# zai-org/SCAIL

Hardware: NVIDIA H100
Metric: denoising steps/sec (SCAIL-14B, 512p/81f) (higher is better)
Workload: dtype bf16

## Files before the change

### scail_b200/csrc/attention.cuh

```cuda
#pragma once
#include "sm90.cuh"

namespace scail {

constexpr int ATT_D = 128;
constexpr int ATT_BQ = 128;
constexpr int ATT_BKV = 128;
constexpr int ATT_STAGES = 2;
constexpr int ATT_TILE_BYTES = 128 * 128 * 2;
constexpr int ATT_HALF_BYTES = ATT_TILE_BYTES / 2;
constexpr int ATT_THREADS = 384;
constexpr int ATT_SMEM_BYTES = (1 + 2 * ATT_STAGES) * ATT_TILE_BYTES + 1024 + 256;
static_assert(ATT_SMEM_BYTES <= 232448, "attention: shared memory budget");

struct AttnParams {
    __nv_bfloat16* out;
    int64_t ldo;
    int q_len;
    int kv_len;
    int kv_off;
    int kv_off1, kv_len1;
    float* o32;
    int64_t ldo32;
    float2* state;
    int heads;
    int q_batch_rows;
    int kv_batch_rows;
    float scale_log2;
    int accumulate;
};


__global__ void __launch_bounds__(ATT_THREADS, 1)
attention_fwd_kernel(const __grid_constant__ CUtensorMap tmap_q, const __grid_constant__ CUtensorMap tmap_k,
                     const __grid_constant__ CUtensorMap tmap_v, const AttnParams p) {
    extern __shared__ uint8_t smem_raw[];
    const uint32_t smem_base = (smem_u32(smem_raw) + 1023u) & ~1023u;
    const uint32_t q_smem = smem_base;
    const uint32_t k_smem = smem_base + ATT_TILE_BYTES;
    const uint32_t v_smem = k_smem + ATT_STAGES * ATT_TILE_BYTES;
    const uint32_t bar_base = v_smem + ATT_STAGES * ATT_TILE_BYTES;
    enum {
        B_QFULL = 0,
        B_KFULL = 1,
        B_KEMPTY = B_KFULL + ATT_STAGES,
        B_VFULL = B_KEMPTY + ATT_STAGES,
        B_VEMPTY = B_VFULL + ATT_STAGES,
        B_COUNT = B_VEMPTY + ATT_STAGES
    };
    static_assert(8 * B_COUNT <= 256, "attention: barrier area");
    auto bar = [&](int i) { return bar_base + 8u * i; };

    const int warp = threadIdx.x >> 5;
    const int lane = threadIdx.x & 31;
    const int head = blockIdx.y;
    const int batch = blockIdx.z;
    const int q0 = blockIdx.x * ATT_BQ;
    const int n_kv0 = (p.kv_len + ATT_BKV - 1) / ATT_BKV;
    const int n_kv = n_kv0 + (p.kv_len1 + ATT_BKV - 1) / ATT_BKV;

    if (warp == 0 && lane == 0) {
        tma_prefetch_desc(&tmap_q);
        tma_prefetch_desc(&tmap_k);
        tma_prefetch_desc(&tmap_v);
        mbar_init(bar(B_QFULL), 1);
        for (int s = 0; s < ATT_STAGES; ++s) {
            mbar_init(bar(B_KFULL + s), 1);
            mbar_init(bar(B_KEMPTY + s), 2);
            mbar_init(bar(B_VFULL + s), 1);
            mbar_init(bar(B_VEMPTY + s), 2);
        }
        fence_barrier_init();
    }
    __syncthreads();

    if (warp < 4) {
        setmaxnreg_dec<40>();
        if (warp == 0 && lane == 0) {
            const int col = head * ATT_D;
            mbar_expect_tx(bar(B_QFULL), ATT_TILE_BYTES);
            for (int h = 0; h < 2; ++h)
                tma_load_2d(q_smem + h * ATT_HALF_BYTES, &tmap_q, bar(B_QFULL), col + h * 64, batch * p.q_batch_rows + q0);
            const int kvbase = batch * p.kv_batch_rows;
            auto kv_row = [&](int j) { return kvbase + (j < n_kv0 ? p.kv_off + j * ATT_BKV : p.kv_off1 + (j - n_kv0) * ATT_BKV); };
            for (int j = 0; j < n_kv; ++j) {
                const int s = j % ATT_STAGES;
                const uint32_t par = ((j / ATT_STAGES) & 1) ^ 1;
                mbar_wait(bar(B_KEMPTY + s), par, 10);
                mbar_expect_tx(bar(B_KFULL + s), ATT_TILE_BYTES);
                for (int h = 0; h < 2; ++h)
                    tma_load_2d(k_smem + s * ATT_TILE_BYTES + h * ATT_HALF_BYTES, &tmap_k, bar(B_KFULL + s), col + h * 64, kv_row(j));
                mbar_wait(bar(B_VEMPTY + s), par, 11);
                mbar_expect_tx(bar(B_VFULL + s), ATT_TILE_BYTES);
                for (int h = 0; h < 2; ++h)
                    tma_load_2d(v_smem + s * ATT_TILE_BYTES + h * ATT_HALF_BYTES, &tmap_v, bar(B_VFULL + s), col + h * 64, kv_row(j));
            }
        }
    } else {
        setmaxnreg_inc<232>();
        const int wg = (warp >> 2) - 1;
        const int t = threadIdx.x & 127;
        const bool releaser = t == 0;
        const int quad = t & 3;
        float m_run[2] = {-INFINITY, -INFINITY};
        float l_run[2] = {0.f, 0.f};
        float o[ATT_D / 2];
#pragma unroll
        for (int i = 0; i < ATT_D / 2; ++i) o[i] = 0.f;
        const uint64_t q_desc = wgmma_desc_kmajor_sw128(q_smem + wg * (64 * 128));
        mbar_wait(bar(B_QFULL), 0, 20);
#pragma unroll 1
        for (int j = 0; j < n_kv; ++j) {
            const int s = j % ATT_STAGES;
            const uint32_t par = (j / ATT_STAGES) & 1;
            const int valid = j < n_kv0 ? min(ATT_BKV, p.kv_len - j * ATT_BKV) : min(ATT_BKV, p.kv_len1 - (j - n_kv0) * ATT_BKV);
            float sc[ATT_BKV / 2];
            mbar_wait(bar(B_KFULL + s), par, 21);
            const uint64_t k_desc = wgmma_desc_kmajor_sw128(k_smem + s * ATT_TILE_BYTES);
            wgmma_fence();
#pragma unroll
            for (int k = 0; k < 8; ++k) {
                const uint64_t off = ((k >> 2) * ATT_HALF_BYTES + (k & 3) * 32) >> 4;
                wgmma_ss<ATT_BKV>(sc, q_desc + off, k_desc + off, k != 0);
            }
            wgmma_commit();
            wgmma_wait<0>();
            fence_regs(sc);
            if (releaser) mbar_arrive(bar(B_KEMPTY + s));
            if (valid < ATT_BKV) {
#pragma unroll
                for (int c = 0; c < ATT_BKV / 8; ++c) {
                    const int col = 8 * c + 2 * quad;
                    if (col >= valid) { sc[4 * c] = -INFINITY; sc[4 * c + 2] = -INFINITY; }
                    if (col + 1 >= valid) { sc[4 * c + 1] = -INFINITY; sc[4 * c + 3] = -INFINITY; }
                }
            }
            float alpha[2], neg_m[2];
#pragma unroll
            for (int h = 0; h < 2; ++h) {
                float mx = -INFINITY;
#pragma unroll
                for (int c = 0; c < ATT_BKV / 8; ++c) mx = fmaxf(mx, fmaxf(sc[4 * c + 2 * h], sc[4 * c + 2 * h + 1]));
                mx = fmaxf(mx, __shfl_xor_sync(0xffffffffu, mx, 1));
                mx = fmaxf(mx, __shfl_xor_sync(0xffffffffu, mx, 2));
                const float m_new = fmaxf(m_run[h], mx * p.scale_log2);
                alpha[h] = fast_exp2(m_run[h] - m_new);
                m_run[h] = m_new;
                l_run[h] *= alpha[h];
                neg_m[h] = -m_new;
            }
#pragma unroll
            for (int c = 0; c < ATT_D / 8; ++c) {
                o[4 * c] *= alpha[0];
                o[4 * c + 1] *= alpha[0];
                o[4 * c + 2] *= alpha[1];
                o[4 * c + 3] *= alpha[1];
            }
            uint32_t pa[ATT_BKV / 16][4];
#pragma unroll
            for (int c = 0; c < ATT_BKV / 8; ++c) {
                float e[4];
#pragma unroll
                for (int i = 0; i < 4; ++i) {
                    e[i] = fast_exp2(fmaf(sc[4 * c + i], p.scale_log2, neg_m[i >> 1]));
                    l_run[i >> 1] += e[i];
                }
                pa[c >> 1][(c & 1) * 2] = pack_bf16(e[0], e[1]);
                pa[c >> 1][(c & 1) * 2 + 1] = pack_bf16(e[2], e[3]);
            }
            mbar_wait(bar(B_VFULL + s), par, 22);
            const uint64_t v_desc = wgmma_desc_mnmajor_sw128(v_smem + s * ATT_TILE_BYTES, ATT_HALF_BYTES);
            fence_regs(o);
            wgmma_fence();
#pragma unroll
            for (int k = 0; k < ATT_BKV / 16; ++k) wgmma_rs_tb<ATT_D>(o, pa[k], v_desc + k * (2048 >> 4));
            wgmma_commit();
            wgmma_wait<0>();
            fence_regs(o);
            if (releaser) mbar_arrive(bar(B_VEMPTY + s));
        }
#pragma unroll
        for (int h = 0; h < 2; ++h) {
            l_run[h] += __shfl_xor_sync(0xffffffffu, l_run[h], 1);
            l_run[h] += __shfl_xor_sync(0xffffffffu, l_run[h], 2);
        }
#pragma unroll
        for (int h = 0; h < 2; ++h) {
            const int qi = q0 + wg * 64 + (t >> 5) * 16 + ((t & 31) >> 2) + 8 * h;
            if (qi >= p.q_len) continue;
            const float inv_l = 1.0f / l_run[h];
            const int64_t grow = static_cast<int64_t>(batch) * p.q_batch_rows + qi;
            if (p.o32 != nullptr) {
                if (quad == 0) p.state[grow * p.heads + head] = make_float2(m_run[h], l_run[h]);
                float* dst = p.o32 + grow * p.ldo32 + head * ATT_D + 2 * quad;
#pragma unroll
                for (int c = 0; c < ATT_D / 8; ++c)
                    *reinterpret_cast<float2*>(dst + 8 * c) = make_float2(o[4 * c + 2 * h] * inv_l, o[4 * c + 2 * h + 1] * inv_l);
                continue;
            }
            __nv_bfloat16* dst = p.out + grow * p.ldo + head * ATT_D + 2 * quad;
#pragma unroll
            for (int c = 0; c < ATT_D / 8; ++c) {
                float f0 = o[4 * c + 2 * h] * inv_l, f1 = o[4 * c + 2 * h + 1] * inv_l;
                uint32_t* d32 = reinterpret_cast<uint32_t*>(dst + 8 * c);
                if (p.accumulate) {
                    const float2 prev = unpack_bf16(*d32);
                    f0 += prev.x;
                    f1 += prev.y;
                }
                *d32 = pack_bf16(f0, f1);
            }
        }
    }
}

__global__ void __launch_bounds__(256) attn_merge_kernel(const float* __restrict__ oa, const float2* __restrict__ sa,
                                                         const float* __restrict__ ob, const float2* __restrict__ sb,
                                                         __nv_bfloat16* __restrict__ out, int64_t ld32, int64_t ldo, int64_t rows,
                                                         int heads) {
    const int64_t item = (static_cast<int64_t>(blockIdx.x) * blockDim.x + threadIdx.x) >> 5;
    if (item >= rows * heads) return;
    const int lane = threadIdx.x & 31;
    const int64_t row = item / heads;
    const int head = static_cast<int>(item - row * heads);
    const float2 a = sa[item], b = sb[item];
    const float m = fmaxf(a.x, b.x);
    const float wa = a.y * fast_exp2(a.x - m), wb = b.y * fast_exp2(b.x - m);
    const float inv = 1.0f / (wa + wb);
    const float ca = wa * inv, cb = wb * inv;
    const float4 va = *reinterpret_cast<const float4*>(oa + row * ld32 + head * ATT_D + lane * 4);
    const float4 vb = *reinterpret_cast<const float4*>(ob + row * ld32 + head * ATT_D + lane * 4);
    uint2 o;
    o.x = pack_bf16(ca * va.x + cb * vb.x, ca * va.y + cb * vb.y);
    o.y = pack_bf16(ca * va.z + cb * vb.z, ca * va.w + cb * vb.w);
    *reinterpret_cast<uint2*>(out + row * ldo + head * ATT_D + lane * 4) = o;
}

}
```

### scail_b200/csrc/sm90.cuh

```cuda
#pragma once
#include <cuda.h>
#include <cuda_bf16.h>
#include <cuda_runtime.h>
#include <stdint.h>
#include <stdio.h>

namespace scail {

__device__ __forceinline__ uint32_t smem_u32(const void* p) {
    return static_cast<uint32_t>(__cvta_generic_to_shared(p));
}

__device__ __forceinline__ uint64_t global_timer_ns() {
    uint64_t t;
    asm volatile("mov.u64 %0, %%globaltimer;" : "=l"(t));
    return t;
}

__device__ __forceinline__ void mbar_init(uint32_t bar, uint32_t count) {
    asm volatile("mbarrier.init.shared::cta.b64 [%0], %1;" ::"r"(bar), "r"(count));
}
__device__ __forceinline__ void fence_barrier_init() {
    asm volatile("fence.mbarrier_init.release.cluster;" ::: "memory");
}
__device__ __forceinline__ void mbar_expect_tx(uint32_t bar, uint32_t bytes) {
    asm volatile("mbarrier.arrive.expect_tx.shared::cta.b64 _, [%0], %1;" ::"r"(bar), "r"(bytes) : "memory");
}
__device__ __forceinline__ void mbar_arrive(uint32_t bar) {
    asm volatile("mbarrier.arrive.shared::cta.b64 _, [%0];" ::"r"(bar) : "memory");
}
__device__ __forceinline__ bool mbar_try_wait(uint32_t bar, uint32_t parity) {
    uint32_t done;
    asm volatile(
        "{\n\t.reg .pred p;\n\t"
        "mbarrier.try_wait.parity.shared::cta.b64 p, [%1], %2;\n\t"
        "selp.b32 %0, 1, 0, p;\n\t}"
        : "=r"(done) : "r"(bar), "r"(parity) : "memory");
    return done != 0;
}
#ifndef SCAIL_MBAR_TIMEOUT_NS
#define SCAIL_MBAR_TIMEOUT_NS 4000000000ull
#endif
__device__ __forceinline__ void mbar_wait(uint32_t bar, uint32_t parity, int tag = 0) {
    if (mbar_try_wait(bar, parity)) return;
    uint64_t t0 = 0;
    uint32_t it = 0;
    while (!mbar_try_wait(bar, parity)) {
        if ((++it & 0x3ff) == 0) {
            uint64_t now = global_timer_ns();
            if (t0 == 0) t0 = now;
            else if (now - t0 > SCAIL_MBAR_TIMEOUT_NS) {
#ifdef SCAIL_MBAR_DEBUG
                printf("scail: mbarrier timeout tag=%d block=(%d,%d,%d) thread=%d parity=%u\n", tag, blockIdx.x,
                       blockIdx.y, blockIdx.z, threadIdx.x, parity);
#endif
                __trap();
            }
        }
    }
}

__device__ __forceinline__ void tma_prefetch_desc(const CUtensorMap* m) {
    asm volatile("prefetch.tensormap [%0];" ::"l"(reinterpret_cast<uint64_t>(m)) : "memory");
}
__device__ __forceinline__ void tma_load_2d(uint32_t dst, const CUtensorMap* m, uint32_t bar, int c0, int c1) {
    asm volatile(
        "cp.async.bulk.tensor.2d.shared::cluster.global.mbarrier::complete_tx::bytes [%0], [%1, {%3, %4}], [%2];"
        ::"r"(dst), "l"(reinterpret_cast<uint64_t>(m)), "r"(bar), "r"(c0), "r"(c1) : "memory");
}
__device__ __forceinline__ void tma_load_4d(uint32_t dst, const CUtensorMap* m, uint32_t bar, int c0, int c1, int c2,
                                            int c3) {
    asm volatile(
        "cp.async.bulk.tensor.4d.shared::cluster.global.mbarrier::complete_tx::bytes [%0], [%1, {%3, %4, %5, %6}], [%2];"
        ::"r"(dst), "l"(reinterpret_cast<uint64_t>(m)), "r"(bar), "r"(c0), "r"(c1), "r"(c2), "r"(c3) : "memory");
}
__device__ __forceinline__ void tma_store_2d(const CUtensorMap* m, uint32_t src, int c0, int c1) {
    asm volatile("cp.async.bulk.tensor.2d.global.shared::cta.bulk_group [%0, {%2, %3}], [%1];"
                 ::"l"(reinterpret_cast<uint64_t>(m)), "r"(src), "r"(c0), "r"(c1) : "memory");
}
__device__ __forceinline__ void bulk_commit() { asm volatile("cp.async.bulk.commit_group;" ::: "memory"); }
__device__ __forceinline__ void bulk_wait_read_all() { asm volatile("cp.async.bulk.wait_group.read 0;" ::: "memory"); }
__device__ __forceinline__ void bulk_wait_all() { asm volatile("cp.async.bulk.wait_group 0;" ::: "memory"); }
__device__ __forceinline__ void fence_proxy_async_smem() { asm volatile("fence.proxy.async.shared::cta;" ::: "memory"); }
__device__ __forceinline__ uint32_t lds_u32(uint32_t a) {
    uint32_t v;
    asm volatile("ld.shared.b32 %0, [%1];" : "=r"(v) : "r"(a) : "memory");
    return v;
}
__device__ __forceinline__ float2 lds_f2(uint32_t a) {
    float2 v;
    asm volatile("ld.shared.v2.f32 {%0, %1}, [%2];" : "=f"(v.x), "=f"(v.y) : "r"(a) : "memory");
    return v;
}
__device__ __forceinline__ void sts_u32(uint32_t a, uint32_t v) {
    asm volatile("st.shared.b32 [%0], %1;" ::"r"(a), "r"(v) : "memory");
}
__device__ __forceinline__ void sts_f2(uint32_t a, float x, float y) {
    asm volatile("st.shared.v2.f32 [%0], {%1, %2};" ::"r"(a), "f"(x), "f"(y) : "memory");
}

__device__ __forceinline__ uint64_t wgmma_desc_kmajor_sw128(uint32_t smem_addr) {
    uint64_t d = 0;
    d |= static_cast<uint64_t>((smem_addr & 0x3FFFFu) >> 4);
    d |= static_cast<uint64_t>(1) << 16;
    d |= static_cast<uint64_t>(1024 >> 4) << 32;
    d |= static_cast<uint64_t>(1) << 62;
    return d;
}
__device__ __forceinline__ uint64_t wgmma_desc_mnmajor_sw128(uint32_t smem_addr, uint32_t lbo_bytes) {
    uint64_t d = 0;
    d |= static_cast<uint64_t>((smem_addr & 0x3FFFFu) >> 4);
    d |= static_cast<uint64_t>((lbo_bytes >> 4) & 0x3FFFu) << 16;
    d |= static_cast<uint64_t>(1024 >> 4) << 32;
    d |= static_cast<uint64_t>(1) << 62;
    return d;
}
__device__ __forceinline__ void wgmma_fence() { asm volatile("wgmma.fence.sync.aligned;" ::: "memory"); }
__device__ __forceinline__ void wgmma_commit() { asm volatile("wgmma.commit_group.sync.aligned;" ::: "memory"); }
template <int N>
__device__ __forceinline__ void wgmma_wait() { asm volatile("wgmma.wait_group.sync.aligned %0;" ::"n"(N) : "memory"); }
template <int R>
__device__ __forceinline__ void fence_regs(float (&d)[R]) {
#pragma unroll
    for (int i = 0; i < R; ++i) asm volatile("" : "+f"(d[i])::"memory");
}

template <int N>
__device__ __forceinline__ void wgmma_ss(float (&d)[N / 2], uint64_t a, uint64_t b, int scale_d);
template <int N>
__device__ __forceinline__ void wgmma_rs_tb(float (&d)[N / 2], const uint32_t (&a)[4], uint64_t b);
template <>
__device__ __forceinline__ void wgmma_ss<16>(float (&d)[8], uint64_t a, uint64_t b, int scale_d) {
    asm volatile(
        "{\n\t.reg .pred p;\n\tsetp.ne.b32 p, %10, 0;\n\t"
        "wgmma.mma_async.sync.aligned.m64n16k16.f32.bf16.bf16 {%0, %1, %2, %3, %4, %5, %6, %7}, %8, %9, p, 1, 1, 0, 0;\n\t}"
        : "+f"(d[0]), "+f"(d[1]), "+f"(d[2]), "+f"(d[3]), "+f"(d[4]), "+f"(d[5]), "+f"(d[6]), "+f"(d[7])
        : "l"(a), "l"(b), "r"(scale_d));
}
template <>
__device__ __forceinline__ void wgmma_ss<96>(float (&d)[48], uint64_t a, uint64_t b, int scale_d) {
    asm volatile(
        "{\n\t.reg .pred p;\n\tsetp.ne.b32 p, %50, 0;\n\t"
        "wgmma.mma_async.sync.aligned.m64n96k16.f32.bf16.bf16 {%0, %1, %2, %3, %4, %5, %6, %7, %8, %9, %10, %11, %12, %13, %14, %15, %16, %17, %18, %19, %20, %21, %22, %23, %24, %25, %26, %27, %28, %29, %30, %31, %32, %33, %34, %35, %36, %37, %38, %39, %40, %41, %42, %43, %44, %45, %46, %47}, %48, %49, p, 1, 1, 0, 0;\n\t}"
        : "+f"(d[0]), "+f"(d[1]), "+f"(d[2]), "+f"(d[3]), "+f"(d[4]), "+f"(d[5]), "+f"(d[6]), "+f"(d[7]), "+f"(d[8]), "+f"(d[9]), "+f"(d[10]), "+f"(d[11]), "+f"(d[12]), "+f"(d[13]), "+f"(d[14]), "+f"(d[15]), "+f"(d[16]), "+f"(d[17]), "+f"(d[18]), "+f"(d[19]), "+f"(d[20]), "+f"(d[21]), "+f"(d[22]), "+f"(d[23]), "+f"(d[24]), "+f"(d[25]), "+f"(d[26]), "+f"(d[27]), "+f"(d[28]), "+f"(d[29]), "+f"(d[30]), "+f"(d[31]), "+f"(d[32]), "+f"(d[33]), "+f"(d[34]), "+f"(d[35]), "+f"(d[36]), "+f"(d[37]), "+f"(d[38]), "+f"(d[39]), "+f"(d[40]), "+f"(d[41]), "+f"(d[42]), "+f"(d[43]), "+f"(d[44]), "+f"(d[45]), "+f"(d[46]), "+f"(d[47])
        : "l"(a), "l"(b), "r"(scale_d));
}
template <>
__device__ __forceinline__ void wgmma_ss<128>(float (&d)[64], uint64_t a, uint64_t b, int scale_d) {
    asm volatile(
        "{\n\t.reg .pred p;\n\tsetp.ne.b32 p, %66, 0;\n\t"
        "wgmma.mma_async.sync.aligned.m64n128k16.f32.bf16.bf16 {%0, %1, %2, %3, %4, %5, %6, %7, %8, %9, %10, %11, %12, %13, %14, %15, %16, %17, %18, %19, %20, %21, %22, %23, %24, %25, %26, %27, %28, %29, %30, %31, %32, %33, %34, %35, %36, %37, %38, %39, %40, %41, %42, %43, %44, %45, %46, %47, %48, %49, %50, %51, %52, %53, %54, %55, %56, %57, %58, %59, %60, %61, %62, %63}, %64, %65, p, 1, 1, 0, 0;\n\t}"
        : "+f"(d[0]), "+f"(d[1]), "+f"(d[2]), "+f"(d[3]), "+f"(d[4]), "+f"(d[5]), "+f"(d[6]), "+f"(d[7]), "+f"(d[8]), "+f"(d[9]), "+f"(d[10]), "+f"(d[11]), "+f"(d[12]), "+f"(d[13]), "+f"(d[14]), "+f"(d[15]), "+f"(d[16]), "+f"(d[17]), "+f"(d[18]), "+f"(d[19]), "+f"(d[20]), "+f"(d[21]), "+f"(d[22]), "+f"(d[23]), "+f"(d[24]), "+f"(d[25]), "+f"(d[26]), "+f"(d[27]), "+f"(d[28]), "+f"(d[29]), "+f"(d[30]), "+f"(d[31]), "+f"(d[32]), "+f"(d[33]), "+f"(d[34]), "+f"(d[35]), "+f"(d[36]), "+f"(d[37]), "+f"(d[38]), "+f"(d[39]), "+f"(d[40]), "+f"(d[41]), "+f"(d[42]), "+f"(d[43]), "+f"(d[44]), "+f"(d[45]), "+f"(d[46]), "+f"(d[47]), "+f"(d[48]), "+f"(d[49]), "+f"(d[50]), "+f"(d[51]), "+f"(d[52]), "+f"(d[53]), "+f"(d[54]), "+f"(d[55]), "+f"(d[56]), "+f"(d[57]), "+f"(d[58]), "+f"(d[59]), "+f"(d[60]), "+f"(d[61]), "+f"(d[62]), "+f"(d[63])
        : "l"(a), "l"(b), "r"(scale_d));
}
template <>
__device__ __forceinline__ void wgmma_ss<192>(float (&d)[96], uint64_t a, uint64_t b, int scale_d) {
    asm volatile(
        "{\n\t.reg .pred p;\n\tsetp.ne.b32 p, %98, 0;\n\t"
        "wgmma.mma_async.sync.aligned.m64n192k16.f32.bf16.bf16 {%0, %1, %2, %3, %4, %5, %6, %7, %8, %9, %10, %11, %12, %13, %14, %15, %16, %17, %18, %19, %20, %21, %22, %23, %24, %25, %26, %27, %28, %29, %30, %31, %32, %33, %34, %35, %36, %37, %38, %39, %40, %41, %42, %43, %44, %45, %46, %47, %48, %49, %50, %51, %52, %53, %54, %55, %56, %57, %58, %59, %60, %61, %62, %63, %64, %65, %66, %67, %68, %69, %70, %71, %72, %73, %74, %75, %76, %77, %78, %79, %80, %81, %82, %83, %84, %85, %86, %87, %88, %89, %90, %91, %92, %93, %94, %95}, %96, %97, p, 1, 1, 0, 0;\n\t}"
        : "+f"(d[0]), "+f"(d[1]), "+f"(d[2]), "+f"(d[3]), "+f"(d[4]), "+f"(d[5]), "+f"(d[6]), "+f"(d[7]), "+f"(d[8]), "+f"(d[9]), "+f"(d[10]), "+f"(d[11]), "+f"(d[12]), "+f"(d[13]), "+f"(d[14]), "+f"(d[15]), "+f"(d[16]), "+f"(d[17]), "+f"(d[18]), "+f"(d[19]), "+f"(d[20]), "+f"(d[21]), "+f"(d[22]), "+f"(d[23]), "+f"(d[24]), "+f"(d[25]), "+f"(d[26]), "+f"(d[27]), "+f"(d[28]), "+f"(d[29]), "+f"(d[30]), "+f"(d[31]), "+f"(d[32]), "+f"(d[33]), "+f"(d[34]), "+f"(d[35]), "+f"(d[36]), "+f"(d[37]), "+f"(d[38]), "+f"(d[39]), "+f"(d[40]), "+f"(d[41]), "+f"(d[42]), "+f"(d[43]), "+f"(d[44]), "+f"(d[45]), "+f"(d[46]), "+f"(d[47]), "+f"(d[48]), "+f"(d[49]), "+f"(d[50]), "+f"(d[51]), "+f"(d[52]), "+f"(d[53]), "+f"(d[54]), "+f"(d[55]), "+f"(d[56]), "+f"(d[57]), "+f"(d[58]), "+f"(d[59]), "+f"(d[60]), "+f"(d[61]), "+f"(d[62]), "+f"(d[63]), "+f"(d[64]), "+f"(d[65]), "+f"(d[66]), "+f"(d[67]), "+f"(d[68]), "+f"(d[69]), "+f"(d[70]), "+f"(d[71]), "+f"(d[72]), "+f"(d[73]), "+f"(d[74]), "+f"(d[75]), "+f"(d[76]), "+f"(d[77]), "+f"(d[78]), "+f"(d[79]), "+f"(d[80]), "+f"(d[81]), "+f"(d[82]), "+f"(d[83]), "+f"(d[84]), "+f"(d[85]), "+f"(d[86]), "+f"(d[87]), "+f"(d[88]), "+f"(d[89]), "+f"(d[90]), "+f"(d[91]), "+f"(d[92]), "+f"(d[93]), "+f"(d[94]), "+f"(d[95])
        : "l"(a), "l"(b), "r"(scale_d));
}
template <>
__device__ __forceinline__ void wgmma_ss<256>(float (&d)[128], uint64_t a, uint64_t b, int scale_d) {
    asm volatile(
        "{\n\t.reg .pred p;\n\tsetp.ne.b32 p, %130, 0;\n\t"
        "wgmma.mma_async.sync.aligned.m64n256k16.f32.bf16.bf16 {%0, %1, %2, %3, %4, %5, %6, %7, %8, %9, %10, %11, %12, %13, %14, %15, %16, %17, %18, %19, %20, %21, %22, %23, %24, %25, %26, %27, %28, %29, %30, %31, %32, %33, %34, %35, %36, %37, %38, %39, %40, %41, %42, %43, %44, %45, %46, %47, %48, %49, %50, %51, %52, %53, %54, %55, %56, %57, %58, %59, %60, %61, %62, %63, %64, %65, %66, %67, %68, %69, %70, %71, %72, %73, %74, %75, %76, %77, %78, %79, %80, %81, %82, %83, %84, %85, %86, %87, %88, %89, %90, %91, %92, %93, %94, %95, %96, %97, %98, %99, %100, %101, %102, %103, %104, %105, %106, %107, %108, %109, %110, %111, %112, %113, %114, %115, %116, %117, %118, %119, %120, %121, %122, %123, %124, %125, %126, %127}, %128, %129, p, 1, 1, 0, 0;\n\t}"
        : "+f"(d[0]), "+f"(d[1]), "+f"(d[2]), "+f"(d[3]), "+f"(d[4]), "+f"(d[5]), "+f"(d[6]), "+f"(d[7]), "+f"(d[8]), "+f"(d[9]), "+f"(d[10]), "+f"(d[11]), "+f"(d[12]), "+f"(d[13]), "+f"(d[14]), "+f"(d[15]), "+f"(d[16]), "+f"(d[17]), "+f"(d[18]), "+f"(d[19]), "+f"(d[20]), "+f"(d[21]), "+f"(d[22]), "+f"(d[23]), "+f"(d[24]), "+f"(d[25]), "+f"(d[26]), "+f"(d[27]), "+f"(d[28]), "+f"(d[29]), "+f"(d[30]), "+f"(d[31]), "+f"(d[32]), "+f"(d[33]), "+f"(d[34]), "+f"(d[35]), "+f"(d[36]), "+f"(d[37]), "+f"(d[38]), "+f"(d[39]), "+f"(d[40]), "+f"(d[41]), "+f"(d[42]), "+f"(d[43]), "+f"(d[44]), "+f"(d[45]), "+f"(d[46]), "+f"(d[47]), "+f"(d[48]), "+f"(d[49]), "+f"(d[50]), "+f"(d[51]), "+f"(d[52]), "+f"(d[53]), "+f"(d[54]), "+f"(d[55]), "+f"(d[56]), "+f"(d[57]), "+f"(d[58]), "+f"(d[59]), "+f"(d[60]), "+f"(d[61]), "+f"(d[62]), "+f"(d[63]), "+f"(d[64]), "+f"(d[65]), "+f"(d[66]), "+f"(d[67]), "+f"(d[68]), "+f"(d[69]), "+f"(d[70]), "+f"(d[71]), "+f"(d[72]), "+f"(d[73]), "+f"(d[74]), "+f"(d[75]), "+f"(d[76]), "+f"(d[77]), "+f"(d[78]), "+f"(d[79]), "+f"(d[80]), "+f"(d[81]), "+f"(d[82]), "+f"(d[83]), "+f"(d[84]), "+f"(d[85]), "+f"(d[86]), "+f"(d[87]), "+f"(d[88]), "+f"(d[89]), "+f"(d[90]), "+f"(d[91]), "+f"(d[92]), "+f"(d[93]), "+f"(d[94]), "+f"(d[95]), "+f"(d[96]), "+f"(d[97]), "+f"(d[98]), "+f"(d[99]), "+f"(d[100]), "+f"(d[101]), "+f"(d[102]), "+f"(d[103]), "+f"(d[104]), "+f"(d[105]), "+f"(d[106]), "+f"(d[107]), "+f"(d[108]), "+f"(d[109]), "+f"(d[110]), "+f"(d[111]), "+f"(d[112]), "+f"(d[113]), "+f"(d[114]), "+f"(d[115]), "+f"(d[116]), "+f"(d[117]), "+f"(d[118]), "+f"(d[119]), "+f"(d[120]), "+f"(d[121]), "+f"(d[122]), "+f"(d[123]), "+f"(d[124]), "+f"(d[125]), "+f"(d[126]), "+f"(d[127])
        : "l"(a), "l"(b), "r"(scale_d));
}
template <>
__device__ __forceinline__ void wgmma_rs_tb<128>(float (&d)[64], const uint32_t (&a)[4], uint64_t b) {
    asm volatile(
        "wgmma.mma_async.sync.aligned.m64n128k16.f32.bf16.bf16 {%0, %1, %2, %3, %4, %5, %6, %7, %8, %9, %10, %11, %12, %13, %14, %15, %16, %17, %18, %19, %20, %21, %22, %23, %24, %25, %26, %27, %28, %29, %30, %31, %32, %33, %34, %35, %36, %37, %38, %39, %40, %41, %42, %43, %44, %45, %46, %47, %48, %49, %50, %51, %52, %53, %54, %55, %56, %57, %58, %59, %60, %61, %62, %63}, {%64, %65, %66, %67}, %68, 1, 1, 1, 1;"
        : "+f"(d[0]), "+f"(d[1]), "+f"(d[2]), "+f"(d[3]), "+f"(d[4]), "+f"(d[5]), "+f"(d[6]), "+f"(d[7]), "+f"(d[8]), "+f"(d[9]), "+f"(d[10]), "+f"(d[11]), "+f"(d[12]), "+f"(d[13]), "+f"(d[14]), "+f"(d[15]), "+f"(d[16]), "+f"(d[17]), "+f"(d[18]), "+f"(d[19]), "+f"(d[20]), "+f"(d[21]), "+f"(d[22]), "+f"(d[23]), "+f"(d[24]), "+f"(d[25]), "+f"(d[26]), "+f"(d[27]), "+f"(d[28]), "+f"(d[29]), "+f"(d[30]), "+f"(d[31]), "+f"(d[32]), "+f"(d[33]), "+f"(d[34]), "+f"(d[35]), "+f"(d[36]), "+f"(d[37]), "+f"(d[38]), "+f"(d[39]), "+f"(d[40]), "+f"(d[41]), "+f"(d[42]), "+f"(d[43]), "+f"(d[44]), "+f"(d[45]), "+f"(d[46]), "+f"(d[47]), "+f"(d[48]), "+f"(d[49]), "+f"(d[50]), "+f"(d[51]), "+f"(d[52]), "+f"(d[53]), "+f"(d[54]), "+f"(d[55]), "+f"(d[56]), "+f"(d[57]), "+f"(d[58]), "+f"(d[59]), "+f"(d[60]), "+f"(d[61]), "+f"(d[62]), "+f"(d[63])
        : "r"(a[0]), "r"(a[1]), "r"(a[2]), "r"(a[3]), "l"(b));
}

__device__ __forceinline__ uint32_t pack_bf16(float lo, float hi) {
    __nv_bfloat162 v = __floats2bfloat162_rn(lo, hi);
    return *reinterpret_cast<uint32_t*>(&v);
}
__device__ __forceinline__ float2 unpack_bf16(uint32_t v) {
    __nv_bfloat162 b = *reinterpret_cast<__nv_bfloat162*>(&v);
    return __bfloat1622float2(b);
}
__device__ __forceinline__ float fast_exp2(float x) {
    float y;
    asm("ex2.approx.ftz.f32 %0, %1;" : "=f"(y) : "f"(x));
    return y;
}
__device__ __forceinline__ uint64_t pack_f32x2(float lo, float hi) {
    uint64_t r;
    asm("mov.b64 %0, {%1, %2};" : "=l"(r) : "f"(lo), "f"(hi));
    return r;
}
__device__ __forceinline__ void unpack_f32x2(uint64_t v, float& lo, float& hi) {
    asm("mov.b64 {%0, %1}, %2;" : "=f"(lo), "=f"(hi) : "l"(v));
}
__device__ __forceinline__ uint64_t fma_f32x2(uint64_t a, uint64_t b, uint64_t c) {
    float a0, a1, b0, b1, c0, c1;
    unpack_f32x2(a, a0, a1);
    unpack_f32x2(b, b0, b1);
    unpack_f32x2(c, c0, c1);
    return pack_f32x2(__fmaf_rn(a0, b0, c0), __fmaf_rn(a1, b1, c1));
}
__device__ __forceinline__ uint64_t add_f32x2(uint64_t a, uint64_t b) {
    float a0, a1, b0, b1;
    unpack_f32x2(a, a0, a1);
    unpack_f32x2(b, b0, b1);
    return pack_f32x2(__fadd_rn(a0, b0), __fadd_rn(a1, b1));
}
template <int N>
__device__ __forceinline__ void setmaxnreg_inc() { asm volatile("setmaxnreg.inc.sync.aligned.u32 %0;" ::"n"(N)); }
template <int N>
__device__ __forceinline__ void setmaxnreg_dec() { asm volatile("setmaxnreg.dec.sync.aligned.u32 %0;" ::"n"(N)); }

__device__ __forceinline__ float fast_tanh(float x) {
    float y;
    asm("tanh.approx.f32 %0, %1;" : "=f"(y) : "f"(x));
    return y;
}
__device__ __forceinline__ float gelu_tanh(float x) {
    const float k0 = 0.7978845608028654f, k1 = 0.044715f;
    float u = k0 * (x + k1 * x * x * x);
    return 0.5f * x * (1.0f + fast_tanh(u));
}
__device__ __forceinline__ void named_bar_sync(int id, int nthreads) {
    asm volatile("bar.sync %0, %1;" ::"r"(id), "r"(nthreads) : "memory");
}

}
```

Before: 0.2251.

## Software-pipeline QK and PV wgmma with ping-pong warpgroup scheduling in attention

Restructures the attention consumer loop so the QK^T wgmma for tile j is issued together with the PV wgmma for tile j-1. Softmax of the current tile then overlaps with tensor-core work. Named barriers make the two consumer warpgroups alternate their MMA issue (FA3-style ping-pong), and the KV pipeline grows from two to three stages to give the producer more slack. This adds register pressure (sc and pa are live across iterations), uses more shared memory, and adds barrier-protocol complexity that could deadlock if the arrive counts are wrong.

```diff
diff --git a/scail_b200/csrc/attention.cuh b/scail_b200/csrc/attention.cuh
--- a/scail_b200/csrc/attention.cuh
+++ b/scail_b200/csrc/attention.cuh
@@ -6,7 +6,7 @@
 constexpr int ATT_D = 128;
 constexpr int ATT_BQ = 128;
 constexpr int ATT_BKV = 128;
-constexpr int ATT_STAGES = 2;
+constexpr int ATT_STAGES = 3;
 constexpr int ATT_TILE_BYTES = 128 * 128 * 2;
 constexpr int ATT_HALF_BYTES = ATT_TILE_BYTES / 2;
 constexpr int ATT_THREADS = 384;
@@ -108,25 +108,26 @@
 #pragma unroll
         for (int i = 0; i < ATT_D / 2; ++i) o[i] = 0.f;
         const uint64_t q_desc = wgmma_desc_kmajor_sw128(q_smem + wg * (64 * 128));
-        mbar_wait(bar(B_QFULL), 0, 20);
-#pragma unroll 1
-        for (int j = 0; j < n_kv; ++j) {
-            const int s = j % ATT_STAGES;
-            const uint32_t par = (j / ATT_STAGES) & 1;
-            const int valid = j < n_kv0 ? min(ATT_BKV, p.kv_len - j * ATT_BKV) : min(ATT_BKV, p.kv_len1 - (j - n_kv0) * ATT_BKV);
-            float sc[ATT_BKV / 2];
-            mbar_wait(bar(B_KFULL + s), par, 21);
-            const uint64_t k_desc = wgmma_desc_kmajor_sw128(k_smem + s * ATT_TILE_BYTES);
-            wgmma_fence();
+        float sc[ATT_BKV / 2];
+        uint32_t pa[ATT_BKV / 16][4];
+        float alpha[2];
+        auto issue_qk = [&](int j) {
+            const uint64_t k_desc = wgmma_desc_kmajor_sw128(k_smem + (j % ATT_STAGES) * ATT_TILE_BYTES);
 #pragma unroll
             for (int k = 0; k < 8; ++k) {
                 const uint64_t off = ((k >> 2) * ATT_HALF_BYTES + (k & 3) * 32) >> 4;
                 wgmma_ss<ATT_BKV>(sc, q_desc + off, k_desc + off, k != 0);
             }
             wgmma_commit();
-            wgmma_wait<0>();
-            fence_regs(sc);
-            if (releaser) mbar_arrive(bar(B_KEMPTY + s));
+        };
+        auto issue_pv = [&](int j) {
+            const uint64_t v_desc = wgmma_desc_mnmajor_sw128(v_smem + (j % ATT_STAGES) * ATT_TILE_BYTES, ATT_HALF_BYTES);
+#pragma unroll
+            for (int k = 0; k < ATT_BKV / 16; ++k) wgmma_rs_tb<ATT_D>(o, pa[k], v_desc + k * (2048 >> 4));
+            wgmma_commit();
+        };
+        auto softmax = [&](int j) {
+            const int valid = j < n_kv0 ? min(ATT_BKV, p.kv_len - j * ATT_BKV) : min(ATT_BKV, p.kv_len1 - (j - n_kv0) * ATT_BKV);
             if (valid < ATT_BKV) {
 #pragma unroll
                 for (int c = 0; c < ATT_BKV / 8; ++c) {
@@ -135,7 +136,7 @@
                     if (col + 1 >= valid) { sc[4 * c + 1] = -INFINITY; sc[4 * c + 3] = -INFINITY; }
                 }
             }
-            float alpha[2], neg_m[2];
+            float neg_m[2];
 #pragma unroll
             for (int h = 0; h < 2; ++h) {
                 float mx = -INFINITY;
@@ -150,35 +151,72 @@
                 neg_m[h] = -m_new;
             }
 #pragma unroll
+            for (int c = 0; c < ATT_BKV / 8; ++c) {
+#pragma unroll
+                for (int i = 0; i < 4; ++i) {
+                    sc[4 * c + i] = fast_exp2(fmaf(sc[4 * c + i], p.scale_log2, neg_m[i >> 1]));
+                    l_run[i >> 1] += sc[4 * c + i];
+                }
+            }
+        };
+        auto rescale_and_pack = [&]() {
+#pragma unroll
             for (int c = 0; c < ATT_D / 8; ++c) {
                 o[4 * c] *= alpha[0];
                 o[4 * c + 1] *= alpha[0];
                 o[4 * c + 2] *= alpha[1];
                 o[4 * c + 3] *= alpha[1];
             }
-            uint32_t pa[ATT_BKV / 16][4];
 #pragma unroll
             for (int c = 0; c < ATT_BKV / 8; ++c) {
-                float e[4];
-#pragma unroll
-                for (int i = 0; i < 4; ++i) {
-                    e[i] = fast_exp2(fmaf(sc[4 * c + i], p.scale_log2, neg_m[i >> 1]));
-                    l_run[i >> 1] += e[i];
-                }
-                pa[c >> 1][(c & 1) * 2] = pack_bf16(e[0], e[1]);
-                pa[c >> 1][(c & 1) * 2 + 1] = pack_bf16(e[2], e[3]);
-            }
-            mbar_wait(bar(B_VFULL + s), par, 22);
-            const uint64_t v_desc = wgmma_desc_mnmajor_sw128(v_smem + s * ATT_TILE_BYTES, ATT_HALF_BYTES);
+                pa[c >> 1][(c & 1) * 2] = pack_bf16(sc[4 * c], sc[4 * c + 1]);
+                pa[c >> 1][(c & 1) * 2 + 1] = pack_bf16(sc[4 * c + 2], sc[4 * c + 3]);
+            }
+        };
+        const int bar_mine = 1 + wg, bar_other = 2 - wg;
+        auto end_turn = [&](int j) { named_bar_arrive_if(bar_other, 256, wg == 0 || j + 1 < n_kv); };
+        bool landed = true;
+        auto wait = [&](uint32_t b, uint32_t par, int tag) { landed = landed && mbar_wait_bounded(b, par, tag); };
+        named_bar_arrive_if(bar_mine, 256, wg == 0);
+        wait(bar(B_QFULL), 0, 20);
+        wait(bar(B_KFULL), 0, 21);
+        named_bar_sync(bar_mine, 256);
+        wgmma_fence();
+        issue_qk(0);
+        end_turn(0);
+        wgmma_wait<0>();
+        fence_regs(sc);
+        mbar_arrive_if(bar(B_KEMPTY), releaser);
+        softmax(0);
+        rescale_and_pack();
+#pragma unroll 1
+        for (int j = 1; j < n_kv; ++j) {
+            const int s = j % ATT_STAGES;
+            wait(bar(B_KFULL + s), (j / ATT_STAGES) & 1, 21);
+            wait(bar(B_VFULL + (j - 1) % ATT_STAGES), ((j - 1) / ATT_STAGES) & 1, 22);
+            named_bar_sync(bar_mine, 256);
             fence_regs(o);
             wgmma_fence();
-#pragma unroll
-            for (int k = 0; k < ATT_BKV / 16; ++k) wgmma_rs_tb<ATT_D>(o, pa[k], v_desc + k * (2048 >> 4));
-            wgmma_commit();
+            issue_qk(j);
+            issue_pv(j - 1);
+            end_turn(j);
+            wgmma_wait<1>();
+            fence_regs(sc);
+            mbar_arrive_if(bar(B_KEMPTY + s), releaser);
+            softmax(j);
             wgmma_wait<0>();
             fence_regs(o);
-            if (releaser) mbar_arrive(bar(B_VEMPTY + s));
-        }
+            mbar_arrive_if(bar(B_VEMPTY + (j - 1) % ATT_STAGES), releaser);
+            rescale_and_pack();
+        }
+        wait(bar(B_VFULL + (n_kv - 1) % ATT_STAGES), ((n_kv - 1) / ATT_STAGES) & 1, 22);
+        fence_regs(o);
+        wgmma_fence();
+        issue_pv(n_kv - 1);
+        wgmma_wait<0>();
+        fence_regs(o);
+        mbar_arrive_if(bar(B_VEMPTY + (n_kv - 1) % ATT_STAGES), releaser);
+        if (!landed) __trap();
 #pragma unroll
         for (int h = 0; h < 2; ++h) {
             l_run[h] += __shfl_xor_sync(0xffffffffu, l_run[h], 1);
diff --git a/scail_b200/csrc/sm90.cuh b/scail_b200/csrc/sm90.cuh
--- a/scail_b200/csrc/sm90.cuh
+++ b/scail_b200/csrc/sm90.cuh
@@ -29,6 +29,10 @@
 __device__ __forceinline__ void mbar_arrive(uint32_t bar) {
     asm volatile("mbarrier.arrive.shared::cta.b64 _, [%0];" ::"r"(bar) : "memory");
 }
+__device__ __forceinline__ void mbar_arrive_if(uint32_t bar, bool pred) {
+    asm volatile("{\n\t.reg .pred p;\n\tsetp.ne.b32 p, %1, 0;\n\t@p mbarrier.arrive.shared::cta.b64 _, [%0];\n\t}"
+                 ::"r"(bar), "r"(static_cast<uint32_t>(pred)) : "memory");
+}
 __device__ __forceinline__ bool mbar_try_wait(uint32_t bar, uint32_t parity) {
     uint32_t done;
     asm volatile(
@@ -41,8 +45,8 @@
 #ifndef SCAIL_MBAR_TIMEOUT_NS
 #define SCAIL_MBAR_TIMEOUT_NS 4000000000ull
 #endif
-__device__ __forceinline__ void mbar_wait(uint32_t bar, uint32_t parity, int tag = 0) {
-    if (mbar_try_wait(bar, parity)) return;
+__device__ __forceinline__ bool mbar_wait_bounded(uint32_t bar, uint32_t parity, int tag = 0) {
+    if (mbar_try_wait(bar, parity)) return true;
     uint64_t t0 = 0;
     uint32_t it = 0;
     while (!mbar_try_wait(bar, parity)) {
@@ -54,10 +58,14 @@
                 printf("scail: mbarrier timeout tag=%d block=(%d,%d,%d) thread=%d parity=%u\n", tag, blockIdx.x,
                        blockIdx.y, blockIdx.z, threadIdx.x, parity);
 #endif
-                __trap();
+                return false;
             }
         }
     }
+    return true;
+}
+__device__ __forceinline__ void mbar_wait(uint32_t bar, uint32_t parity, int tag = 0) {
+    if (!mbar_wait_bounded(bar, parity, tag)) __trap();
 }
 
 __device__ __forceinline__ void tma_prefetch_desc(const CUtensorMap* m) {
@@ -229,5 +237,9 @@
 __device__ __forceinline__ void named_bar_sync(int id, int nthreads) {
     asm volatile("bar.sync %0, %1;" ::"r"(id), "r"(nthreads) : "memory");
 }
-
-}
+__device__ __forceinline__ void named_bar_arrive_if(int id, int nthreads, bool pred) {
+    asm volatile("{\n\t.reg .pred p;\n\tsetp.ne.b32 p, %2, 0;\n\t@p bar.arrive %0, %1;\n\t}"
+                 ::"r"(id), "r"(nthreads), "r"(static_cast<uint32_t>(pred)) : "memory");
+}
+
+}
```

Measured after the change: 0.2298, median of 6. +2.1%, better.
